# lucidrains/transfusion-pytorch

Measured on NVIDIA H100. Metric: train tokens/sec (text+latent) at d=512 L=8 seq=1024, higher is better.
Workload: dtype bf16

## Files before the change

transfusion_pytorch_b200/csrc/gemm_sm90.cuh:

```cuda
#pragma once
#include "sm90_ptx.cuh"
#include "dropout.cuh"

namespace tfx {

constexpr int GEMM_BM = 128;
constexpr int GEMM_BN = 128;
constexpr int GEMM_BK = 64;
constexpr int GEMM_UK = 16;

enum : int { EPI_STORE = 0, EPI_QKVG = 1, EPI_RESID = 2, EPI_GEGLU = 3, EPI_GEGLU_DROP = 4, EPI_QKVG_ROPE = 5 };

struct GemmParams {
  int M, N, K;
  int k_splits;
  float* out_f32; long long ld_f32;
  __nv_bfloat16* out_bf16; long long ld_bf16;
  const float* bias;
  const long long* row_off;
  float alpha;
  int accumulate_f32;
  int K1;
  int H;
  __nv_bfloat16 *q, *k, *v;
  float* gates;
  float* mix_pre;
  float* qk_inv;
  const float *q_gamma, *k_gamma;
  const int* rope_pos;
  const float2* rope_cs;
  int rope_len;
  const int* kv_rows;
  const float* x_res; float* x_out; __nv_bfloat16* x_out_bf16;
  __nv_bfloat16* y_bf16;
  const int* cond_row;
  const float* zgate;
  long long zgate_ld;
  const float* ls;
  __nv_bfloat16* vg;
  __nv_bfloat16* h;
  DropParams drop;
};

template <int EPI> struct GemmCfg {
  static constexpr int BM = GEMM_BM;
  static constexpr int THREADS = 384;
  static constexpr int STAGES = 4;
  static constexpr int A_BYTES = GEMM_BM * GEMM_BK * 2;
  static constexpr int B_BYTES = GEMM_BN * GEMM_BK * 2;
  static constexpr int STAGE_BYTES = A_BYTES + B_BYTES;
  static constexpr int ACC_BYTES = GEMM_BM * GEMM_BN * 4;
  static constexpr int STG_WARP = EPI == 2 ? 4096 + 2048 : 4096;
  static constexpr int STAGING = (EPI == EPI_GEGLU || EPI == EPI_GEGLU_DROP ? 8 : 4) * STG_WARP;
  static constexpr int SMEM_BYTES = STAGES * STAGE_BYTES + ACC_BYTES + STAGING + 1024  + 256 ;
  static_assert(SMEM_BYTES <= 227 * 1024, "shared memory of one block");
};

__device__ __forceinline__ uint32_t acc_off(int r, int col) { return r * 512 + ((((col >> 2) ^ (r & 7))) << 4) + (col & 3) * 4; }
__device__ __forceinline__ void acc_ld32(const uint8_t* acc, int r, int col, uint32_t (&v)[32]) {
#pragma unroll
  for (int q = 0; q < 8; ++q) {
    const uint4 t = *reinterpret_cast<const uint4*>(acc + r * 512 + ((((col >> 2) + q) ^ (r & 7)) << 4));
    v[4 * q] = t.x; v[4 * q + 1] = t.y; v[4 * q + 2] = t.z; v[4 * q + 3] = t.w;
  }
}

__device__ __forceinline__ void gelu_parts(float g, float& cdf, float& pdf) {
  const float ax = fabsf(g) * 0.70710678118654752f;
  const float t = __fdividef(1.f, fmaf(0.3275911f, ax, 1.f));
  const float E = __expf(-ax * ax);
  float poly = fmaf(1.061405429f, t, -1.453152027f);
  poly = fmaf(poly, t, 1.421413741f);
  poly = fmaf(poly, t, -0.284496736f);
  poly = fmaf(poly, t, 0.254829592f);
  const float h = 0.5f * poly * t * E;
  cdf = g >= 0.f ? 1.f - h : h;
  pdf = 0.3989422804014327f * E;
}
__device__ __forceinline__ float gelu_erf(float x) { float c, d; gelu_parts(x, c, d); return x * c; }
__device__ __forceinline__ float2 geglu_pair(float2 g, float2 v) {
  return make_float2(gelu_erf(g.x) * v.x, gelu_erf(g.y) * v.y);
}

__device__ __forceinline__ void cp_async16_zfill(void* smem, const void* gmem, bool valid) {
  const int sz = valid ? 16 : 0;
  asm volatile("cp.async.cg.shared.global [%0], [%1], 16, %2;" ::"r"(smem_u32(smem)), "l"(gmem), "r"(sz) : "memory");
}

__device__ __forceinline__ uint32_t pack_bf16(float a, float b) {
  __nv_bfloat162 t = __floats2bfloat162_rn(a, b);
  return *reinterpret_cast<uint32_t*>(&t);
}
__device__ __forceinline__ float2 unpack2_bf16_(uint32_t w) {
  __nv_bfloat162 t = *reinterpret_cast<__nv_bfloat162*>(&w);
  return __bfloat1622float2(t);
}

template <int CH>
__device__ __forceinline__ void stg_put(uint8_t* sw, int lane, const uint32_t* w) {
#pragma unroll
  for (int c = 0; c < CH; ++c)
    *reinterpret_cast<uint4*>(sw + lane * 128 + ((c ^ (lane & 7)) << 4)) = make_uint4(w[4 * c], w[4 * c + 1], w[4 * c + 2], w[4 * c + 3]);
}
template <int CH>
__device__ __forceinline__ void stg_get(const uint8_t* sw, int lane, uint32_t* w) {
#pragma unroll
  for (int c = 0; c < CH; ++c) {
    const uint4 t = *reinterpret_cast<const uint4*>(sw + lane * 128 + ((c ^ (lane & 7)) << 4));
    w[4 * c] = t.x; w[4 * c + 1] = t.y; w[4 * c + 2] = t.z; w[4 * c + 3] = t.w;
  }
}
template <int CH>
__device__ __forceinline__ void stg_store(const uint8_t* sw, int lane, uint8_t* g, long long pitch, int rows_valid) {
  constexpr int RPI = 32 / CH;
#pragma unroll
  for (int it = 0; it < 32 / RPI; ++it) {
    const int row = it * RPI + lane / CH, ch = lane % CH;
    if (row < rows_valid)
      *reinterpret_cast<uint4*>(g + row * pitch + ch * 16) = *reinterpret_cast<const uint4*>(sw + row * 128 + ((ch ^ (row & 7)) << 4));
  }
}
__device__ __forceinline__ void stg_fetch(int lane, const uint8_t* g, long long pitch, int rows_valid, uint4 (&t)[8]) {
#pragma unroll
  for (int it = 0; it < 8; ++it) {
    const int row = it * 4 + lane / 8, ch = lane % 8;
    t[it] = row < rows_valid ? *reinterpret_cast<const uint4*>(g + row * pitch + ch * 16) : make_uint4(0, 0, 0, 0);
  }
}
__device__ __forceinline__ void stg_fill(uint8_t* sw, int lane, const uint4 (&t)[8]) {
#pragma unroll
  for (int it = 0; it < 8; ++it) {
    const int row = it * 4 + lane / 8, ch = lane % 8;
    *reinterpret_cast<uint4*>(sw + row * 128 + ((ch ^ (row & 7)) << 4)) = t[it];
  }
}

__device__ __forceinline__ void stg_put_pack(uint8_t* sw, int lane, const float* y) {
#pragma unroll
  for (int c = 0; c < 4; ++c)
    *reinterpret_cast<uint4*>(sw + lane * 128 + ((c ^ (lane & 7)) << 4)) =
        make_uint4(pack_bf16(y[8 * c], y[8 * c + 1]), pack_bf16(y[8 * c + 2], y[8 * c + 3]), pack_bf16(y[8 * c + 4], y[8 * c + 5]), pack_bf16(y[8 * c + 6], y[8 * c + 7]));
}
__device__ __forceinline__ void stg64_put(uint8_t* sw, int lane, const uint32_t* w) {
#pragma unroll
  for (int c = 0; c < 4; ++c)
    *reinterpret_cast<uint4*>(sw + lane * 64 + ((c ^ ((lane >> 1) & 3)) << 4)) = make_uint4(w[4 * c], w[4 * c + 1], w[4 * c + 2], w[4 * c + 3]);
}
__device__ __forceinline__ void stg64_put_pack(uint8_t* sw, int lane, const float* y) {
#pragma unroll
  for (int c = 0; c < 4; ++c)
    *reinterpret_cast<uint4*>(sw + lane * 64 + ((c ^ ((lane >> 1) & 3)) << 4)) =
        make_uint4(pack_bf16(y[8 * c], y[8 * c + 1]), pack_bf16(y[8 * c + 2], y[8 * c + 3]), pack_bf16(y[8 * c + 4], y[8 * c + 5]), pack_bf16(y[8 * c + 6], y[8 * c + 7]));
}
__device__ __forceinline__ void stg64_store(const uint8_t* sw, int lane, uint8_t* g, long long pitch, int rows_valid) {
#pragma unroll
  for (int it = 0; it < 4; ++it) {
    const int row = it * 8 + (lane >> 2), ch = lane & 3;
    if (row < rows_valid)
      *reinterpret_cast<uint4*>(g + row * pitch + ch * 16) = *reinterpret_cast<const uint4*>(sw + row * 64 + ((ch ^ ((row >> 1) & 3)) << 4));
  }
}

__device__ __forceinline__ void stg64_store_rows(const uint8_t* sw, int lane, uint8_t* g, long long pitch, int rows_valid, const int* __restrict__ rows) {
#pragma unroll
  for (int it = 0; it < 4; ++it) {
    const int row = it * 8 + (lane >> 2), ch = lane & 3;
    if (row < rows_valid)
      *reinterpret_cast<uint4*>(g + (long long)rows[row] * pitch + ch * 16) = *reinterpret_cast<const uint4*>(sw + row * 64 + ((ch ^ ((row >> 1) & 3)) << 4));
  }
}
template <int CH>
__device__ __forceinline__ void stg_store_rows(const uint8_t* sw, int lane, uint8_t* g, long long pitch, int rows_valid, const int* __restrict__ rows) {
  constexpr int RPI = 32 / CH;
#pragma unroll
  for (int it = 0; it < 32 / RPI; ++it) {
    const int row = it * RPI + lane / CH, ch = lane % CH;
    if (row < rows_valid)
      *reinterpret_cast<uint4*>(g + (long long)rows[row] * pitch + ch * 16) = *reinterpret_cast<const uint4*>(sw + row * 128 + ((ch ^ (row & 7)) << 4));
  }
}

template <class RowOf>
__device__ __forceinline__ void store_slice(const GemmParams& p, uint8_t* sw, int lane, uint32_t (&r)[32], int cbase, RowOf row_of) {
  const bool f32_staged = p.out_f32 && (p.row_off || (p.ld_f32 & 3) == 0) && ((reinterpret_cast<uintptr_t>(p.out_f32) & 15) == 0);
  const bool bf16_staged = p.out_bf16 && (p.ld_bf16 & 7) == 0 && ((reinterpret_cast<uintptr_t>(p.out_bf16) & 15) == 0);
  const int row = row_of(lane);
  const bool row_ok = row < p.M;
  const bool full = cbase + 32 <= p.N;
  float v[32];
#pragma unroll
  for (int j = 0; j < 32; ++j) v[j] = __uint_as_float(r[j]);
  if (p.alpha != 1.f) {
#pragma unroll
    for (int j = 0; j < 32; ++j) v[j] *= p.alpha;
  }
  if (p.bias) {
    if (full) {
#pragma unroll
      for (int j = 0; j < 32; j += 4) { const float4 b = *reinterpret_cast<const float4*>(p.bias + cbase + j); v[j] += b.x; v[j + 1] += b.y; v[j + 2] += b.z; v[j + 3] += b.w; }
    } else {
      for (int j = 0; j < 32; ++j) if (cbase + j < p.N) v[j] += p.bias[cbase + j];
    }
  }
  if (p.out_f32) {
    if (full && f32_staged) {
#pragma unroll
      for (int j = 0; j < 32; ++j) r[j] = __float_as_uint(v[j]);
      stg_put<8>(sw, lane, r);
      __syncwarp();
      auto put = [&](float* dst, float x) { if (p.accumulate_f32) atomicAdd(dst, x); else *dst = x; };
#pragma unroll
      for (int it = 0; it < 8; ++it) {
        const int rr = it * 4 + (lane >> 3), ch = lane & 7;
        const int grow = row_of(rr);
        if (grow < p.M) {
          const long long off = p.row_off ? p.row_off[grow] : (long long)grow * p.ld_f32;
          if (off >= 0) {
            float* drow = p.out_f32 + off + cbase;
            const uint8_t* srow = sw + rr * 128;
            const int a = (int)(reinterpret_cast<uintptr_t>(drow) >> 2) & 3;
            if (a == 0) {
              float* dst = drow + ch * 4;
              const float4 t = *reinterpret_cast<const float4*>(srow + ((ch ^ (rr & 7)) << 4));
              if (p.accumulate_f32) asm volatile("red.global.add.v4.f32 [%0], {%1, %2, %3, %4};" ::"l"(dst), "f"(t.x), "f"(t.y), "f"(t.z), "f"(t.w) : "memory");
              else *reinterpret_cast<float4*>(dst) = t;
            } else {
              const int pe = 4 - a;
              auto col = [&](int j) { return *reinterpret_cast<const float*>(srow + (((j >> 2) ^ (rr & 7)) << 4) + (j & 3) * 4); };
              if (ch < 7) {
                const int j = pe + 4 * ch;
                float* dst = drow + j;
                const float4 t = make_float4(col(j), col(j + 1), col(j + 2), col(j + 3));
                if (p.accumulate_f32) asm volatile("red.global.add.v4.f32 [%0], {%1, %2, %3, %4};" ::"l"(dst), "f"(t.x), "f"(t.y), "f"(t.z), "f"(t.w) : "memory");
                else *reinterpret_cast<float4*>(dst) = t;
              } else {
#pragma unroll
                for (int i = 0; i < 4; ++i) { const int j = i < pe ? i : 28 + i; put(drow + j, col(j)); }
              }
            }
          }
        }
      }
      __syncwarp();
    } else if (row_ok) {
      const long long off = p.row_off ? p.row_off[row] : (long long)row * p.ld_f32;
      if (off >= 0) {
        float* dst = p.out_f32 + off + cbase;
        for (int j = 0; j < 32; ++j)
          if (cbase + j < p.N) { if (p.accumulate_f32) atomicAdd(dst + j, v[j]); else dst[j] = v[j]; }
      }
    }
  }
  if (p.out_bf16) {
    if (full && bf16_staged) {
      uint32_t w[16];
#pragma unroll
      for (int j = 0; j < 16; ++j) w[j] = pack_bf16(v[2 * j], v[2 * j + 1]);
      stg_put<4>(sw, lane, w);
      __syncwarp();
#pragma unroll
      for (int it = 0; it < 4; ++it) {
        const int rr = it * 8 + (lane >> 2), ch = lane & 3;
        const int grow = row_of(rr);
        if (grow < p.M)
          *reinterpret_cast<uint4*>(p.out_bf16 + (long long)grow * p.ld_bf16 + cbase + ch * 8) = *reinterpret_cast<const uint4*>(sw + rr * 128 + ((ch ^ (rr & 7)) << 4));
      }
      __syncwarp();
    } else if (row_ok) {
      __nv_bfloat16* dst = p.out_bf16 + (long long)row * p.ld_bf16 + cbase;
      for (int j = 0; j < 32; ++j) if (cbase + j < p.N) dst[j] = __float2bfloat16(v[j]);
    }
  }
}

template <int BM, int CL>
struct GemmSched {
  struct Work { int m_blk, n_blk, kb0, kb1; };
  int n_tiles, unit_items, kb_total, kb_per_split, num_items;
  __device__ __forceinline__ explicit GemmSched(const GemmParams& p) {
    const int m_tiles = (p.M + BM - 1) / BM;
    n_tiles = (p.N + GEMM_BN - 1) / GEMM_BN;
    kb_total = (p.K + GEMM_BK - 1) / GEMM_BK;
    kb_per_split = (kb_total + p.k_splits - 1) / p.k_splits;
    unit_items = (m_tiles + CL - 1) / CL * n_tiles;
    num_items = unit_items * p.k_splits;
  }
  __device__ __forceinline__ Work work(int item, int cta_rank) const {
    const int split = item / unit_items;
    const int rem = item - split * unit_items;
    const int m_unit = rem / n_tiles;
    const int kb0 = split * kb_per_split;
    return {m_unit * CL + cta_rank, rem - m_unit * n_tiles, kb0, min(kb0 + kb_per_split, kb_total)};
  }
};

template <int STAGES>
struct GemmRing {
  int stage = 0; uint32_t phase = 0;
  __device__ __forceinline__ void step() { if (++stage == STAGES) { stage = 0; phase ^= 1; } }
};

template <class Cfg, bool A_MN, bool B_MN, int CL, bool TWO_A>
__device__ __forceinline__ void gemm_fill(uint8_t* smem, uint64_t* full_bar, uint64_t* empty_bar, GemmRing<Cfg::STAGES>& ring,
                                          const CUtensorMap* tmA, const CUtensorMap* tmA2, const CUtensorMap* tmB, const GemmParams& p,
                                          int kb, int m_blk, int n_blk, int cta_rank) {
  constexpr int BM = Cfg::BM, BN = GEMM_BN;
  mbar_wait(&empty_bar[ring.stage], ring.phase ^ 1);
  uint8_t* sA = smem + ring.stage * Cfg::STAGE_BYTES;
  uint8_t* sB = sA + Cfg::A_BYTES;
  uint64_t* bar = &full_bar[ring.stage];
  mbar_expect_tx(bar, Cfg::STAGE_BYTES);
  if (!A_MN) {
    if (!TWO_A || kb * GEMM_BK < p.K1) tma_load_2d(tmA, bar, sA, kb * GEMM_BK, m_blk * BM);
    else tma_load_2d(tmA2, bar, sA, kb * GEMM_BK - p.K1, m_blk * BM);
  } else {
#pragma unroll
    for (int a = 0; a < BM / 64; ++a)
      tma_load_2d(tmA, bar, sA + a * (GEMM_BK * 128), m_blk * BM + a * 64, kb * GEMM_BK);
  }
  if constexpr (CL > 1) {
    if (!B_MN) tma_load_2d_multicast(tmB, bar, sB + cta_rank * (64 * 128), kb * GEMM_BK, n_blk * BN + cta_rank * 64, (uint16_t)3);
    else tma_load_2d_multicast(tmB, bar, sB + cta_rank * (GEMM_BK * 128), n_blk * BN + cta_rank * 64, kb * GEMM_BK, (uint16_t)3);
  } else if (!B_MN) {
    tma_load_2d(tmB, bar, sB, kb * GEMM_BK, n_blk * BN);
  } else {
#pragma unroll
    for (int a = 0; a < BN / 64; ++a)
      tma_load_2d(tmB, bar, sB + a * (GEMM_BK * 128), n_blk * BN + a * 64, kb * GEMM_BK);
  }
  ring.step();
}

template <class Cfg, bool A_MN, bool B_MN, class Release>
__device__ __forceinline__ int gemm_mainloop(uint8_t* smem, uint64_t* full_bar, GemmRing<Cfg::STAGES>& ring, uint32_t a_off, int kb0, int kb1,
                                             float (&d0)[64], float (&d1)[64], Release& release) {
#pragma unroll
  for (int i = 0; i < 64; ++i) { d0[i] = 0.f; d1[i] = 0.f; }
  int prev_stage = -1;
  for (int kb = kb0; kb < kb1; ++kb) {
    mbar_wait(&full_bar[ring.stage], ring.phase);
    const uint32_t sA = smem_u32(smem + ring.stage * Cfg::STAGE_BYTES) + a_off;
    const uint32_t sB = smem_u32(smem + ring.stage * Cfg::STAGE_BYTES) + Cfg::A_BYTES;
    wgmma_reg_fence(d0);
    wgmma_reg_fence(d1);
    wgmma_fence();
#pragma unroll
    for (int k = 0; k < GEMM_BK / GEMM_UK; ++k) {
      const uint64_t db = B_MN ? wgmma_desc_sw128(sB + k * (GEMM_UK * 128), GEMM_BK * 128, 1024)
                               : wgmma_desc_sw128(sB + k * (GEMM_UK * 2), 16, 1024);
      const uint64_t da0 = A_MN ? wgmma_desc_sw128(sA + k * (GEMM_UK * 128), GEMM_BK * 128, 1024)
                                : wgmma_desc_sw128(sA + k * (GEMM_UK * 2), 16, 1024);
      const uint64_t da1 = A_MN ? wgmma_desc_sw128(sA + GEMM_BK * 128 + k * (GEMM_UK * 128), GEMM_BK * 128, 1024)
                                : wgmma_desc_sw128(sA + 64 * 128 + k * (GEMM_UK * 2), 16, 1024);
      const uint32_t acc_flag = (kb > kb0 || k > 0) ? 1u : 0u;
      wgmma_m64n128_ss<A_MN ? 1 : 0, B_MN ? 1 : 0>(d0, da0, db, acc_flag);
      wgmma_m64n128_ss<A_MN ? 1 : 0, B_MN ? 1 : 0>(d1, da1, db, acc_flag);
    }
    wgmma_commit();
    wgmma_wait<1>();
    if (prev_stage >= 0) release(prev_stage);
    prev_stage = ring.stage;
    ring.step();
  }
  return prev_stage;
}

template <class Release>
__device__ __forceinline__ void gemm_drain(float (&d0)[64], float (&d1)[64], int last_stage, Release& release) {
  wgmma_wait<0>();
  wgmma_reg_fence(d0);
  wgmma_reg_fence(d1);
  if (last_stage >= 0) release(last_stage);
}

template <bool A_MN, bool B_MN, int EPI, int CL>
__global__ void __launch_bounds__(384, 1)
gemm_sm90_kernel(const __grid_constant__ CUtensorMap tmA, const __grid_constant__ CUtensorMap tmA2, const __grid_constant__ CUtensorMap tmB, const GemmParams p) {
  using Cfg = GemmCfg<EPI>;
  constexpr bool GEGLU = EPI == EPI_GEGLU || EPI == EPI_GEGLU_DROP;
  constexpr int BN = GEMM_BN;
  constexpr int STAGES = Cfg::STAGES;
  static_assert(Cfg::STAGE_BYTES % 1024 == 0 && 2 * STAGES <= 32, "stage alignment / barrier area");
  extern __shared__ __align__(1024) uint8_t smem_raw[];
  uint8_t* smem = smem_raw;
  if (threadIdx.x == 0 && (smem_u32(smem) & 1023u) != 0) __trap();
  uint8_t* acc = smem + STAGES * Cfg::STAGE_BYTES;
  uint8_t* staging = acc + Cfg::ACC_BYTES;
  uint64_t* bars = reinterpret_cast<uint64_t*>(staging + Cfg::STAGING);
  uint64_t* full_bar = bars;
  uint64_t* empty_bar = bars + STAGES;

  const int warp = threadIdx.x >> 5, lane = threadIdx.x & 31;
  const GemmSched<GEMM_BM, CL> sched(p);
  const int num_items = sched.num_items;
  const int cta_rank = CL > 1 ? (int)cluster_ctarank() : 0;
  const int first_item = blockIdx.x / CL, item_stride = gridDim.x / CL;

  if (threadIdx.x == 0) {
    tma_prefetch_desc(&tmA);
    tma_prefetch_desc(&tmB);
    for (int s = 0; s < STAGES; ++s) { mbar_init(&full_bar[s], 1); mbar_init(&empty_bar[s], 4 * CL); }
    mbar_fence_init();
  }
  __syncthreads();
  if constexpr (CL > 1) cluster_sync_all();

  if (warp < 4) {
    setmaxnreg_dec<40>();
    if (threadIdx.x == 0) {
      GemmRing<STAGES> ring;
      for (int item = first_item; item < num_items; item += item_stride) {
        const auto w = sched.work(item, cta_rank);
        for (int kb = w.kb0; kb < w.kb1; ++kb)
          gemm_fill<Cfg, A_MN, B_MN, CL, true>(smem, full_bar, empty_bar, ring, &tmA, &tmA2, &tmB, p, kb, w.m_blk, w.n_blk, cta_rank);
      }
    }
  } else {
    setmaxnreg_inc<232>();
    constexpr int BAR_TILE = 1, BAR_MMA = 3, BAR_ACC = 5;
    const int cw = (warp >> 2) - 1;
    const int quad = warp & 3;
    uint8_t* sw = staging + ((GEGLU ? 4 * cw : 0) + quad) * Cfg::STG_WARP;
    const int erow = quad * 32 + lane;
    GemmRing<STAGES> ring;
    auto release = [&](int s) {
      __syncwarp();
      if (lane == 0) {
        if constexpr (CL > 1) { mbar_arrive_cluster(&empty_bar[s], 0); mbar_arrive_cluster(&empty_bar[s], 1); }
        else mbar_arrive(&empty_bar[s]);
      }
    };
    int nth = 0;
    for (int item = first_item; item < num_items; item += item_stride, ++nth) {
      const auto [m_blk, n_blk, kb0, kb1] = sched.work(item, cta_rank);
      if ((nth & 1) != cw) {
        const int s = ring.stage + (kb1 - kb0);
        ring.stage = s % STAGES;
        ring.phase ^= (uint32_t)(s / STAGES) & 1u;
        continue;
      }
      const bool has_next = item + item_stride < num_items;
      if (nth > 0) named_bar_sync(BAR_MMA + cw, 256);
      float d0[64], d1[64];
      const int last_stage = gemm_mainloop<Cfg, A_MN, B_MN>(smem, full_bar, ring, 0, kb0, kb1, d0, d1, release);
      if (has_next) named_bar_arrive(BAR_MMA + (cw ^ 1), 256);
      gemm_drain(d0, d1, last_stage, release);

      if (nth > 0) named_bar_sync(BAR_ACC + cw, 256);
      {
        const int r0 = quad * 16 + (lane >> 2);
#pragma unroll
        for (int q = 0; q < 16; ++q) {
          const int c = 8 * q + 2 * (lane & 3);
          *reinterpret_cast<float2*>(acc + acc_off(r0, c)) = make_float2(d0[4 * q], d0[4 * q + 1]);
          *reinterpret_cast<float2*>(acc + acc_off(r0 + 8, c)) = make_float2(d0[4 * q + 2], d0[4 * q + 3]);
          *reinterpret_cast<float2*>(acc + acc_off(r0 + 64, c)) = make_float2(d1[4 * q], d1[4 * q + 1]);
          *reinterpret_cast<float2*>(acc + acc_off(r0 + 72, c)) = make_float2(d1[4 * q + 2], d1[4 * q + 3]);
        }
      }
      named_bar_sync(BAR_TILE + cw, 128);

      const int wrow0 = m_blk * GEMM_BM + quad * 32;
      const int row = wrow0 + lane;
      const bool row_ok = row < p.M;
      const int rows_valid = min(32, p.M - wrow0);
      const int col0 = n_blk * BN;
      int qk_pos = 0;
      if constexpr (EPI == EPI_QKVG || EPI == EPI_QKVG_ROPE) { qk_pos = row_ok ? p.rope_pos[row] : 0; }
      if constexpr (EPI == EPI_RESID) { qk_pos = (row_ok && p.cond_row) ? p.cond_row[row] : -1; }

      if constexpr (EPI == EPI_STORE) {
#pragma unroll 1
        for (int c = 0; c < BN / 32; ++c) {
          const int cbase = col0 + c * 32;
          if (cbase >= p.N) break;
          uint32_t r[32];
          acc_ld32(acc, erow, c * 32, r);
          store_slice(p, sw, lane, r, cbase, [&](int i) { return wrow0 + i; });
        }
      } else if constexpr (EPI == EPI_QKVG || EPI == EPI_QKVG_ROPE) {
        const int tps = p.H >> 1;
        const int kind = n_blk / tps;
        const int tis = n_blk - kind * tps;
        const long long HI = (long long)p.H * 64;
        if (kind <= 1) {
          const float* gamma = kind == 0 ? p.q_gamma : p.k_gamma;
          __nv_bfloat16* dstm = kind == 0 ? p.q : p.k;
          const float2* cs = p.rope_cs + qk_pos;
#pragma unroll
          for (int hh = 0; hh < 2; ++hh) {
            uint32_t r0[32], r1[32];
            acc_ld32(acc, erow, hh * 64, r0);
            acc_ld32(acc, erow, hh * 64 + 32, r1);
            float sc = 1.f;
            if constexpr (EPI == EPI_QKVG) {
              float ss = 0.f;
#pragma unroll
              for (int j = 0; j < 32; ++j) { float a = __uint_as_float(r0[j]), b = __uint_as_float(r1[j]); ss += a * a + b * b; }
              const float inv = 1.f / fmaxf(sqrtf(ss), 1e-12f);
              if (row_ok) p.qk_inv[(long long)row * 2 * p.H + kind * p.H + tis * 2 + hh] = inv;
              sc = inv * 8.f;
            }
            const int head = tis * 2 + hh;
            uint32_t outw[32];
#pragma unroll
            for (int dh = 0; dh < 2; ++dh) {
              uint32_t* rr = dh == 0 ? r0 : r1;
#pragma unroll
              for (int i = 0; i < 16; ++i) {
                const int d0 = dh * 32 + 2 * i;
                float y0 = __uint_as_float(rr[2 * i]), y1 = __uint_as_float(rr[2 * i + 1]);
                if constexpr (EPI == EPI_QKVG) {
                  const float2 gm = *reinterpret_cast<const float2*>(gamma + d0);
                  y0 = y0 * sc * (gm.x + 1.f);
                  y1 = y1 * sc * (gm.y + 1.f);
                }
                const float2 cc = cs[(long long)(dh * 16 + i) * p.rope_len];
                outw[dh * 16 + i] = pack_bf16(y0 * cc.x - y1 * cc.y, y1 * cc.x + y0 * cc.y);
              }
            }
            stg_put<8>(sw, lane, outw);
            __syncwarp();
            if (kind == 1 && p.kv_rows) stg_store_rows<8>(sw, lane, reinterpret_cast<uint8_t*>(dstm + head * 64), HI * 2, rows_valid, p.kv_rows + wrow0);
            else stg_store<8>(sw, lane, reinterpret_cast<uint8_t*>(dstm + (long long)wrow0 * HI + head * 64), HI * 2, rows_valid);
            __syncwarp();
          }
        } else if (kind == 2) {
#pragma unroll
          for (int c = 0; c < 2; ++c) {
            uint32_t r0[32], r1[32], w[32];
            acc_ld32(acc, erow, c * 64, r0);
            acc_ld32(acc, erow, c * 64 + 32, r1);
#pragma unroll
            for (int j = 0; j < 16; ++j) {
              w[j] = pack_bf16(__uint_as_float(r0[2 * j]), __uint_as_float(r0[2 * j + 1]));
              w[16 + j] = pack_bf16(__uint_as_float(r1[2 * j]), __uint_as_float(r1[2 * j + 1]));
            }
            stg_put<8>(sw, lane, w);
            __syncwarp();
            if (p.kv_rows) stg_store_rows<8>(sw, lane, reinterpret_cast<uint8_t*>(p.v + tis * 128 + c * 64), HI * 2, rows_valid, p.kv_rows + wrow0);
            else stg_store<8>(sw, lane, reinterpret_cast<uint8_t*>(p.v + (long long)wrow0 * HI + tis * 128 + c * 64), HI * 2, rows_valid);
            __syncwarp();
          }
        } else {
          uint32_t r[32];
          acc_ld32(acc, erow, 0, r);
          if (row_ok) {
            float* dst = p.gates + (long long)row * p.H;
#pragma unroll
            for (int j = 0; j < 32; ++j) if (j < p.H) dst[j] = __uint_as_float(r[j]);
            if (p.mix_pre) {
              float* dm = p.mix_pre + (long long)row * p.H;
#pragma unroll
              for (int j = 0; j < 32; ++j) if (j >= p.H && j < 2 * p.H) dm[j - p.H] = __uint_as_float(r[j]);
            }
          }
        }
      } else if constexpr (EPI == EPI_RESID) {
        const int crow = qk_pos;
        const float* zrow = (p.zgate && crow >= 0) ? p.zgate + (long long)crow * p.zgate_ld : nullptr;
        uint8_t* swb = sw + 4096;
        uint4 xres[8];
        auto fetch = [&](int sl) {
          stg_fetch(lane, reinterpret_cast<const uint8_t*>(p.x_res + (long long)wrow0 * p.N + col0 + sl * 32), (long long)p.N * 4,
                    col0 + sl * 32 < p.N ? rows_valid : 0, xres);
        };
        fetch(0);
#pragma unroll 1
        for (int sl = 0; sl < BN / 32; ++sl) {
          const int cbase = col0 + sl * 32;
          if (cbase >= p.N) break;
          __syncwarp();
          stg_fill(sw, lane, xres);
          if (sl + 1 < BN / 32) fetch(sl + 1);
          uint32_t r[32];
          acc_ld32(acc, erow, sl * 32, r);
          float y[32];
#pragma unroll
          for (int j = 0; j < 32; ++j) y[j] = __uint_as_float(r[j]);
          if (p.bias) {
#pragma unroll
            for (int j = 0; j < 32; j += 4) { const float4 b = *reinterpret_cast<const float4*>(p.bias + cbase + j); y[j] += b.x; y[j + 1] += b.y; y[j + 2] += b.z; y[j + 3] += b.w; }
          }
          if (p.y_bf16) {
            stg64_put_pack(swb, lane, y);
            __syncwarp();
            stg64_store(swb, lane, reinterpret_cast<uint8_t*>(p.y_bf16 + (long long)wrow0 * p.N + cbase), (long long)p.N * 2, rows_valid);
            __syncwarp();
          }
          {
            uint32_t xrv[32];
            __syncwarp();
            stg_get<8>(sw, lane, xrv);
            if (zrow) {
#pragma unroll
              for (int j = 0; j < 32; j += 4) {
                const float4 s4 = *reinterpret_cast<const float4*>(zrow + cbase + j);
                y[j] = __uint_as_float(xrv[j]) + y[j] * s4.x; y[j + 1] = __uint_as_float(xrv[j + 1]) + y[j + 1] * s4.y;
                y[j + 2] = __uint_as_float(xrv[j + 2]) + y[j + 2] * s4.z; y[j + 3] = __uint_as_float(xrv[j + 3]) + y[j + 3] * s4.w;
              }
            } else if (p.ls) {
#pragma unroll
              for (int j = 0; j < 32; j += 4) {
                const float4 s4 = *reinterpret_cast<const float4*>(p.ls + cbase + j);
                y[j] = __uint_as_float(xrv[j]) + y[j] * (s4.x + 1.f); y[j + 1] = __uint_as_float(xrv[j + 1]) + y[j + 1] * (s4.y + 1.f);
                y[j + 2] = __uint_as_float(xrv[j + 2]) + y[j + 2] * (s4.z + 1.f); y[j + 3] = __uint_as_float(xrv[j + 3]) + y[j + 3] * (s4.w + 1.f);
              }
            } else {
#pragma unroll
              for (int j = 0; j < 32; ++j) y[j] += __uint_as_float(xrv[j]);
            }
          }
          if (p.x_out)
#pragma unroll
          for (int hfc = 0; hfc < 2; ++hfc) {
            uint32_t w16[16];
#pragma unroll
            for (int j = 0; j < 16; ++j) w16[j] = __float_as_uint(y[hfc * 16 + j]);
            __syncwarp();
            stg64_put(swb, lane, w16);
            __syncwarp();
            stg64_store(swb, lane, reinterpret_cast<uint8_t*>(p.x_out + (long long)wrow0 * p.N + cbase + hfc * 16), (long long)p.N * 4, rows_valid);
          }
          if (p.x_out_bf16) {
            __syncwarp();
            stg64_put_pack(swb, lane, y);
            __syncwarp();
            stg64_store(swb, lane, reinterpret_cast<uint8_t*>(p.x_out_bf16 + (long long)wrow0 * p.N + cbase), (long long)p.N * 2, rows_valid);
          }
          __syncwarp();
        }
      } else if constexpr (GEGLU) {
        uint32_t keep[2] = {0u, 0u};
        if constexpr (EPI == EPI_GEGLU_DROP) {
          const uint32_t k0 = __ldg(p.drop.key), k1 = __ldg(p.drop.key + 1);
#pragma unroll
          for (int q = 0; q < 8; ++q) keep[q >> 2] |= drop_keep8(p.drop, k0, k1, DROP_SITE_FFN, 0, (uint32_t)row, (uint32_t)(n_blk * 8 + q)) << (8 * (q & 3));
        }
        uint32_t ra[4][32];
#pragma unroll
        for (int q = 0; q < 4; ++q) acc_ld32(acc, erow, q * 32, ra[q]);
        if (has_next) named_bar_arrive(BAR_ACC + (cw ^ 1), 256);
#pragma unroll
        for (int c = 0; c < 2; ++c) {
          const int cv = col0 + c * 32, cg = cv + 64;
          if (cv >= p.N) break;
          float v[32], g[32];
#pragma unroll
          for (int j = 0; j < 32; ++j) { v[j] = __uint_as_float(ra[c][j]) + p.bias[cv + j]; g[j] = __uint_as_float(ra[2 + c][j]) + p.bias[cg + j]; }
          __syncwarp();
          stg64_put_pack(sw, lane, v);
          __syncwarp();
          stg64_store(sw, lane, reinterpret_cast<uint8_t*>(p.vg + (long long)wrow0 * p.N + cv), (long long)p.N * 2, rows_valid);
          __syncwarp();
          stg64_put_pack(sw, lane, g);
          __syncwarp();
          stg64_store(sw, lane, reinterpret_cast<uint8_t*>(p.vg + (long long)wrow0 * p.N + cg), (long long)p.N * 2, rows_valid);
#pragma unroll
          for (int j = 0; j < 32; j += 2) {
            const float2 o = geglu_pair(make_float2(g[j], g[j + 1]), make_float2(v[j], v[j + 1]));
            g[j] = o.x; g[j + 1] = o.y;
          }
          if constexpr (EPI == EPI_GEGLU_DROP) {
#pragma unroll
            for (int j = 0; j < 32; ++j) g[j] = (keep[c] >> j) & 1u ? g[j] * p.drop.scale : 0.f;
          }
          __syncwarp();
          stg64_put_pack(sw, lane, g);
          __syncwarp();
          stg64_store(sw, lane, reinterpret_cast<uint8_t*>(p.h + (long long)wrow0 * (p.N / 2) + n_blk * 64 + c * 32), (long long)p.N, rows_valid);
          __syncwarp();
        }
      }
      if (!GEGLU && has_next) named_bar_arrive(BAR_ACC + (cw ^ 1), 256);
    }
  }
  if constexpr (CL > 1) {
    __syncthreads();
    cluster_sync_all();
  }
}

struct GemmWideCfg {
  static constexpr int BM = 256;
  static constexpr int THREADS = 384;
  static constexpr int STAGES = 4;
  static constexpr int A_BYTES = BM * GEMM_BK * 2;
  static constexpr int B_BYTES = GEMM_BN * GEMM_BK * 2;
  static constexpr int STAGE_BYTES = A_BYTES + B_BYTES;
  static constexpr int STAGING = 8 * 4096;
  static constexpr int SMEM_BYTES = STAGES * STAGE_BYTES + STAGING + 1024  + 256 ;
  static_assert(SMEM_BYTES <= 227 * 1024, "shared memory of one block");
};

template <bool A_MN, bool B_MN>
__global__ void __launch_bounds__(384, 1)
gemm_sm90_wide_kernel(const __grid_constant__ CUtensorMap tmA, const __grid_constant__ CUtensorMap tmB, const GemmParams p) {
  using Cfg = GemmWideCfg;
  constexpr int BM = Cfg::BM, BN = GEMM_BN, STAGES = Cfg::STAGES;
  static_assert(Cfg::STAGE_BYTES % 1024 == 0, "stage alignment");
  extern __shared__ __align__(1024) uint8_t smem_raw[];
  uint8_t* smem = smem_raw;
  if (threadIdx.x == 0 && (smem_u32(smem) & 1023u) != 0) __trap();
  uint8_t* staging = smem + STAGES * Cfg::STAGE_BYTES;
  uint64_t* full_bar = reinterpret_cast<uint64_t*>(staging + Cfg::STAGING);
  uint64_t* empty_bar = full_bar + STAGES;

  const int warp = threadIdx.x >> 5, lane = threadIdx.x & 31;
  const GemmSched<BM, 1> sched(p);
  const int num_items = sched.num_items;

  if (threadIdx.x == 0) {
    tma_prefetch_desc(&tmA);
    tma_prefetch_desc(&tmB);
    for (int s = 0; s < STAGES; ++s) { mbar_init(&full_bar[s], 1); mbar_init(&empty_bar[s], 8); }
    mbar_fence_init();
  }
  __syncthreads();

  if (warp < 4) {
    setmaxnreg_dec<40>();
    if (threadIdx.x == 0) {
      GemmRing<STAGES> ring;
      for (int item = blockIdx.x; item < num_items; item += gridDim.x) {
        const auto w = sched.work(item, 0);
        for (int kb = w.kb0; kb < w.kb1; ++kb)
          gemm_fill<Cfg, A_MN, B_MN, 1, false>(smem, full_bar, empty_bar, ring, &tmA, nullptr, &tmB, p, kb, w.m_blk, w.n_blk, 0);
      }
    }
  } else {
    setmaxnreg_inc<232>();
    const int cw = (warp >> 2) - 1;
    const int quad = warp & 3;
    uint8_t* sw = staging + (4 * cw + quad) * 4096;
    const uint32_t a_half = (uint32_t)cw * (A_MN ? 2 * GEMM_BK * 128 : 128 * 128);
    GemmRing<STAGES> ring;
    auto release = [&](int s) { __syncwarp(); if (lane == 0) mbar_arrive(&empty_bar[s]); };
    for (int item = blockIdx.x; item < num_items; item += gridDim.x) {
      const auto [m_blk, n_blk, kb0, kb1] = sched.work(item, 0);
      float d0[64], d1[64];
      const int last_stage = gemm_mainloop<Cfg, A_MN, B_MN>(smem, full_bar, ring, a_half, kb0, kb1, d0, d1, release);
      gemm_drain(d0, d1, last_stage, release);

      const int wrow0 = m_blk * BM + 128 * cw + 16 * quad;
      const int r0 = lane >> 2;
#pragma unroll
      for (int c = 0; c < BN / 32; ++c) {
        const int cbase = n_blk * BN + c * 32;
        if (cbase >= p.N) break;
#pragma unroll
        for (int q4 = 0; q4 < 4; ++q4) {
          const int q = 4 * c + q4, col = 8 * q4 + 2 * (lane & 3);
          auto put2 = [&](int rr, float x, float y) {
            *reinterpret_cast<float2*>(sw + rr * 128 + ((((col >> 2) ^ (rr & 7))) << 4) + (col & 3) * 4) = make_float2(x, y);
          };
          put2(r0, d0[4 * q], d0[4 * q + 1]);
          put2(r0 + 8, d0[4 * q + 2], d0[4 * q + 3]);
          put2(r0 + 16, d1[4 * q], d1[4 * q + 1]);
          put2(r0 + 24, d1[4 * q + 2], d1[4 * q + 3]);
        }
        __syncwarp();
        uint32_t r[32];
        stg_get<8>(sw, lane, r);
        __syncwarp();
        store_slice(p, sw, lane, r, cbase, [&](int i) { return wrow0 + (i & 15) + ((i >> 4) << 6); });
      }
    }
  }
}

typedef CUresult (*PFN_encodeTiled)(CUtensorMap*, CUtensorMapDataType, cuuint32_t, void*, const cuuint64_t*, const cuuint64_t*,
                                    const cuuint32_t*, const cuuint32_t*, CUtensorMapInterleave, CUtensorMapSwizzle,
                                    CUtensorMapL2promotion, CUtensorMapFloatOOBfill);

inline PFN_encodeTiled get_encode_fn() {
  static PFN_encodeTiled fn = nullptr;
  if (!fn) {
    void* f = nullptr;
    cudaDriverEntryPointQueryResult qres;
    if (cudaGetDriverEntryPoint("cuTensorMapEncodeTiled", &f, cudaEnableDefault, &qres) != cudaSuccess || !f) return nullptr;
    fn = reinterpret_cast<PFN_encodeTiled>(f);
  }
  return fn;
}

inline int make_tmap_bf16(CUtensorMap* tm, const void* ptr, long long inner, long long outer, long long ld, int box_rows) {
  PFN_encodeTiled enc = get_encode_fn();
  if (!enc) return -1;
  cuuint64_t dims[2] = {(cuuint64_t)inner, (cuuint64_t)outer};
  cuuint64_t strides[1] = {(cuuint64_t)ld * 2};
  cuuint32_t box[2] = {64, (cuuint32_t)box_rows};
  cuuint32_t estr[2] = {1, 1};
  CUresult r = enc(tm, CU_TENSOR_MAP_DATA_TYPE_BFLOAT16, 2, const_cast<void*>(ptr), dims, strides, box, estr,
                   CU_TENSOR_MAP_INTERLEAVE_NONE, CU_TENSOR_MAP_SWIZZLE_128B, CU_TENSOR_MAP_L2_PROMOTION_L2_256B,
                   CU_TENSOR_MAP_FLOAT_OOB_FILL_NONE);
  return r == CUDA_SUCCESS ? 0 : -(int)r - 1000;
}

struct GemmOperand {
  const void* ptr;
  long long ld;
  bool mn_major;
  const void* ptr2 = nullptr;
  long long ld2 = 0;
};

inline int make_operand_tmap(CUtensorMap* tm, const GemmOperand& X, long long mn, long long k, int box_rows) {
  return X.mn_major ? make_tmap_bf16(tm, X.ptr, mn, k, X.ld, GEMM_BK) : make_tmap_bf16(tm, X.ptr, k, mn, X.ld, box_rows);
}

template <class Cfg, auto kern, class... Args>
int launch_persistent(int items, int num_sms, cudaStream_t stream, const Args&... args) {
  static bool attr_set = false;
  if (!attr_set) {
    if (cudaFuncSetAttribute(kern, cudaFuncAttributeMaxDynamicSharedMemorySize, Cfg::SMEM_BYTES) != cudaSuccess) return -2;
    attr_set = true;
  }
  const int grid = items < num_sms ? items : num_sms;
  kern<<<grid, Cfg::THREADS, Cfg::SMEM_BYTES, stream>>>(args...);
  return cudaGetLastError() == cudaSuccess ? 0 : -3;
}

inline int& gemm_cluster_mode_ref() {
  static int mode = -1;
  if (mode < 0) { const char* e = getenv("TFX_GEMM_CLUSTER"); mode = e ? atoi(e) : 1; }
  return mode;
}

inline int gemm_effective_splits(int K, int k_splits) {
  const int kbt = (K + GEMM_BK - 1) / GEMM_BK;
  int s = k_splits < 1 ? 1 : k_splits > kbt ? kbt : k_splits;
  const int per = (kbt + s - 1) / s;
  return (kbt + per - 1) / per;
}
inline int gemm_kb_per_item(int K, int k_splits) { return ((K + GEMM_BK - 1) / GEMM_BK + k_splits - 1) / k_splits; }

constexpr int GEMM_WIDE_MIN_KB = 16;
inline int& gemm_wide_mode_ref() { static int mode = 1; return mode; }
inline bool gemm_store_wide(int K, int k_splits) {
  const int mode = gemm_wide_mode_ref();
  if (mode != 1) return mode == 2;
  return gemm_cluster_mode_ref() == 1 && gemm_kb_per_item(K, gemm_effective_splits(K, k_splits)) >= GEMM_WIDE_MIN_KB;
}

template <bool A_MN, bool B_MN>
int launch_gemm_wide_t(const GemmOperand& A, const GemmOperand& B, const GemmParams& p_in, int num_sms, cudaStream_t stream) {
  using Cfg = GemmWideCfg;
  GemmParams p = p_in;
  p.K1 = p.K;
  p.k_splits = gemm_effective_splits(p.K, p.k_splits);
  const int items = ((p.M + Cfg::BM - 1) / Cfg::BM) * ((p.N + GEMM_BN - 1) / GEMM_BN) * p.k_splits;
  if (items <= 0) return 0;
  CUtensorMap tmA, tmB;
  int rc = make_operand_tmap(&tmA, A, p.M, p.K, Cfg::BM);
  if (rc) return rc;
  rc = make_operand_tmap(&tmB, B, p.N, p.K, GEMM_BN);
  if (rc) return rc;
  return launch_persistent<Cfg, gemm_sm90_wide_kernel<A_MN, B_MN>>(items, num_sms, stream, tmA, tmB, p);
}

template <bool A_MN, bool B_MN, int EPI>
int launch_gemm_t(const GemmOperand& A, const GemmOperand& B, const GemmParams& p_in, int num_sms, cudaStream_t stream) {
  using Cfg = GemmCfg<EPI>;
  GemmParams p = p_in;
  CUtensorMap tmA, tmA2, tmB;
  const bool two = (!A_MN) && A.ptr2 != nullptr;
  if (!two) p.K1 = p.K;
  int rc = make_operand_tmap(&tmA, A, p.M, p.K1, GEMM_BM);
  if (rc) return rc;
  if (two) { rc = make_tmap_bf16(&tmA2, A.ptr2, p.K - p.K1, p.M, A.ld2, GEMM_BM); if (rc) return rc; } else tmA2 = tmA;
  p.k_splits = gemm_effective_splits(p.K, p.k_splits);
  const int m_tiles = (p.M + GEMM_BM - 1) / GEMM_BM, n_tiles = (p.N + GEMM_BN - 1) / GEMM_BN;
  const int items = m_tiles * n_tiles * p.k_splits;
  if (items <= 0) return 0;
  const int mode = gemm_cluster_mode_ref();
  const int kb_item = gemm_kb_per_item(p.K, p.k_splits);
  const bool paired = mode == 2 || (mode == 3 && m_tiles >= 2 && kb_item >= 16 && items >= 2 * num_sms);
  rc = make_operand_tmap(&tmB, B, p.N, p.K, paired ? GEMM_BN / 2 : GEMM_BN);
  if (rc) return rc;
  if (paired) {
    auto kern = gemm_sm90_kernel<A_MN, B_MN, EPI, 2>;
    static int max_clusters = 0;
    cudaLaunchConfig_t cfg;
    memset(&cfg, 0, sizeof(cfg));
    cudaLaunchAttribute at[1];
    at[0].id = cudaLaunchAttributeClusterDimension;
    at[0].val.clusterDim.x = 2; at[0].val.clusterDim.y = 1; at[0].val.clusterDim.z = 1;
    cfg.blockDim = dim3(Cfg::THREADS); cfg.dynamicSmemBytes = Cfg::SMEM_BYTES; cfg.stream = stream; cfg.attrs = at; cfg.numAttrs = 1;
    if (!max_clusters) {
      if (cudaFuncSetAttribute(kern, cudaFuncAttributeMaxDynamicSharedMemorySize, Cfg::SMEM_BYTES) != cudaSuccess) return -2;
      cfg.gridDim = dim3(2 * (num_sms / 2));
      int nc = 0;
      if (cudaOccupancyMaxActiveClusters(&nc, kern, &cfg) != cudaSuccess || nc < 1) { cudaGetLastError(); nc = num_sms / 2; }
      max_clusters = nc < num_sms / 2 ? nc : num_sms / 2;
    }
    const int pair_items = ((m_tiles + 1) / 2) * n_tiles * p.k_splits;
    const int clusters = pair_items < max_clusters ? pair_items : max_clusters;
    cfg.gridDim = dim3(2 * clusters);
    return cudaLaunchKernelEx(&cfg, kern, tmA, tmA2, tmB, p) == cudaSuccess ? 0 : -3;
  }
  return launch_persistent<Cfg, gemm_sm90_kernel<A_MN, B_MN, EPI, 1>>(items, num_sms, stream, tmA, tmA2, tmB, p);
}

}
```

transfusion_pytorch_b200/csrc/sm90_ptx.cuh:

```cuda
#pragma once
#include <cuda.h>
#include <cuda_runtime.h>
#include <cuda_bf16.h>
#include <stdint.h>
#include <stdio.h>

namespace tfx {

#ifndef TFX_SPIN_LIMIT
#define TFX_SPIN_LIMIT (1u << 24)
#endif

__device__ __forceinline__ uint32_t smem_u32(const void* p) {
  return static_cast<uint32_t>(__cvta_generic_to_shared(p));
}

__device__ __forceinline__ void mbar_init(uint64_t* bar, uint32_t count) {
  asm volatile("mbarrier.init.shared::cta.b64 [%0], %1;" ::"r"(smem_u32(bar)), "r"(count));
}
__device__ __forceinline__ void mbar_fence_init() {
  asm volatile("fence.mbarrier_init.release.cluster;" ::: "memory");
}
__device__ __forceinline__ void mbar_expect_tx(uint64_t* bar, uint32_t bytes) {
  asm volatile("mbarrier.arrive.expect_tx.shared::cta.b64 _, [%0], %1;" ::"r"(smem_u32(bar)), "r"(bytes) : "memory");
}
__device__ __forceinline__ void mbar_arrive(uint64_t* bar) {
  asm volatile("mbarrier.arrive.shared::cta.b64 _, [%0];" ::"r"(smem_u32(bar)) : "memory");
}
__device__ __forceinline__ bool mbar_try_wait(uint64_t* bar, uint32_t parity) {
  uint32_t ok;
  asm volatile(
      "{\n\t.reg .pred p;\n\t"
      "mbarrier.try_wait.parity.shared::cta.b64 p, [%1], %2;\n\t"
      "selp.u32 %0, 1, 0, p;\n\t}"
      : "=r"(ok) : "r"(smem_u32(bar)), "r"(parity) : "memory");
  return ok != 0;
}
__device__ __forceinline__ void mbar_wait(uint64_t* bar, uint32_t parity) {
  uint32_t spins = 0;
  while (!mbar_try_wait(bar, parity)) {
    if (++spins > TFX_SPIN_LIMIT) {
#if defined(TFX_DEBUG_SPIN) && TFX_DEBUG_SPIN
      printf("tfx: mbarrier timeout block %d thread %d bar %u parity %u\n", blockIdx.x, threadIdx.x, smem_u32(bar), parity);
#endif
      __trap();
    }
  }
}

__device__ __forceinline__ void tma_prefetch_desc(const CUtensorMap* m) {
  asm volatile("prefetch.tensormap [%0];" ::"l"(reinterpret_cast<uint64_t>(m)) : "memory");
}
__device__ __forceinline__ void tma_load_2d(const CUtensorMap* m, uint64_t* bar, void* smem, int c0, int c1) {
  asm volatile(
      "cp.async.bulk.tensor.2d.shared::cluster.global.mbarrier::complete_tx::bytes [%0], [%1, {%3, %4}], [%2];"
      ::"r"(smem_u32(smem)), "l"(reinterpret_cast<uint64_t>(m)), "r"(smem_u32(bar)), "r"(c0), "r"(c1)
      : "memory");
}
__device__ __forceinline__ void tma_load_1d(const CUtensorMap* m, uint64_t* bar, void* smem, int c0) {
  asm volatile(
      "cp.async.bulk.tensor.1d.shared::cluster.global.mbarrier::complete_tx::bytes [%0], [%1, {%3}], [%2];"
      ::"r"(smem_u32(smem)), "l"(reinterpret_cast<uint64_t>(m)), "r"(smem_u32(bar)), "r"(c0)
      : "memory");
}
__device__ __forceinline__ void tma_reduce_add_2d(const CUtensorMap* m, const void* smem, int c0, int c1) {
  asm volatile("cp.reduce.async.bulk.tensor.2d.global.shared::cta.add.tile.bulk_group [%0, {%2, %3}], [%1];"
               ::"l"(reinterpret_cast<uint64_t>(m)), "r"(smem_u32(smem)), "r"(c0), "r"(c1) : "memory");
}
__device__ __forceinline__ void bulk_commit() { asm volatile("cp.async.bulk.commit_group;" ::: "memory"); }
__device__ __forceinline__ void bulk_wait_read_all() { asm volatile("cp.async.bulk.wait_group.read 0;" ::: "memory"); }
__device__ __forceinline__ void bulk_wait_all() { asm volatile("cp.async.bulk.wait_group 0;" ::: "memory"); }
__device__ __forceinline__ void tma_load_2d_multicast(const CUtensorMap* m, uint64_t* bar, void* smem, int c0, int c1, uint16_t mask) {
  asm volatile(
      "cp.async.bulk.tensor.2d.shared::cluster.global.mbarrier::complete_tx::bytes.multicast::cluster [%0], [%1, {%3, %4}], [%2], %5;"
      ::"r"(smem_u32(smem)), "l"(reinterpret_cast<uint64_t>(m)), "r"(smem_u32(bar)), "r"(c0), "r"(c1), "h"(mask)
      : "memory");
}
__device__ __forceinline__ uint32_t cluster_ctarank() { uint32_t r; asm volatile("mov.u32 %0, %%cluster_ctarank;" : "=r"(r)); return r; }
__device__ __forceinline__ void cluster_sync_all() {
  asm volatile("barrier.cluster.arrive.release.aligned;\n\tbarrier.cluster.wait.acquire.aligned;" ::: "memory");
}
__device__ __forceinline__ void mbar_arrive_cluster(uint64_t* bar, uint32_t rank) {
  uint32_t remote;
  asm volatile("mapa.shared::cluster.u32 %0, %1, %2;" : "=r"(remote) : "r"(smem_u32(bar)), "r"(rank));
  asm volatile("mbarrier.arrive.release.cluster.shared::cluster.b64 _, [%0];" ::"r"(remote) : "memory");
}
__device__ __forceinline__ void fence_proxy_async_smem() {
  asm volatile("fence.proxy.async.shared::cta;" ::: "memory");
}
__device__ __forceinline__ void named_bar_sync(int id, int count) {
  asm volatile("bar.sync %0, %1;" ::"r"(id), "r"(count) : "memory");
}
__device__ __forceinline__ void named_bar_arrive(int id, int count) {
  asm volatile("bar.arrive %0, %1;" ::"r"(id), "r"(count) : "memory");
}

template <int N> __device__ __forceinline__ void setmaxnreg_dec() { asm volatile("setmaxnreg.dec.sync.aligned.u32 %0;" ::"n"(N)); }
template <int N> __device__ __forceinline__ void setmaxnreg_inc() { asm volatile("setmaxnreg.inc.sync.aligned.u32 %0;" ::"n"(N)); }

__device__ __forceinline__ void wgmma_fence() { asm volatile("wgmma.fence.sync.aligned;" ::: "memory"); }
__device__ __forceinline__ void wgmma_commit() { asm volatile("wgmma.commit_group.sync.aligned;" ::: "memory"); }
template <int N> __device__ __forceinline__ void wgmma_wait() { asm volatile("wgmma.wait_group.sync.aligned %0;" ::"n"(N) : "memory"); }
template <int N> __device__ __forceinline__ void wgmma_reg_fence(float (&d)[N]) {
#pragma unroll
  for (int i = 0; i < N; ++i) asm volatile("" : "+f"(d[i])::"memory");
}

template <int TA, int TB>
__device__ __forceinline__ void wgmma_m64n128_ss(float (&d)[64], uint64_t da, uint64_t db, uint32_t accumulate) {
  asm volatile(
      "{\n\t.reg .pred p;\n\t"
      "setp.ne.b32 p, %66, 0;\n\t"
      "wgmma.mma_async.sync.aligned.m64n128k16.f32.bf16.bf16 "
      "{%0, %1, %2, %3, %4, %5, %6, %7, %8, %9, %10, %11, %12, %13, %14, %15, %16, %17, %18, %19, %20, %21, %22, %23, %24, %25, %26, %27, %28, %29, %30, %31, %32, %33, %34, %35, %36, %37, %38, %39, %40, %41, %42, %43, %44, %45, %46, %47, %48, %49, %50, %51, %52, %53, %54, %55, %56, %57, %58, %59, %60, %61, %62, %63}, "
      "%64, %65, p, 1, 1, %67, %68;\n\t}"
      : "+f"(d[0]), "+f"(d[1]), "+f"(d[2]), "+f"(d[3]), "+f"(d[4]), "+f"(d[5]), "+f"(d[6]), "+f"(d[7]), "+f"(d[8]), "+f"(d[9]), "+f"(d[10]), "+f"(d[11]), "+f"(d[12]), "+f"(d[13]), "+f"(d[14]), "+f"(d[15]), "+f"(d[16]), "+f"(d[17]), "+f"(d[18]), "+f"(d[19]), "+f"(d[20]), "+f"(d[21]), "+f"(d[22]), "+f"(d[23]), "+f"(d[24]), "+f"(d[25]), "+f"(d[26]), "+f"(d[27]), "+f"(d[28]), "+f"(d[29]), "+f"(d[30]), "+f"(d[31]), "+f"(d[32]), "+f"(d[33]), "+f"(d[34]), "+f"(d[35]), "+f"(d[36]), "+f"(d[37]), "+f"(d[38]), "+f"(d[39]), "+f"(d[40]), "+f"(d[41]), "+f"(d[42]), "+f"(d[43]), "+f"(d[44]), "+f"(d[45]), "+f"(d[46]), "+f"(d[47]), "+f"(d[48]), "+f"(d[49]), "+f"(d[50]), "+f"(d[51]), "+f"(d[52]), "+f"(d[53]), "+f"(d[54]), "+f"(d[55]), "+f"(d[56]), "+f"(d[57]), "+f"(d[58]), "+f"(d[59]), "+f"(d[60]), "+f"(d[61]), "+f"(d[62]), "+f"(d[63])
      : "l"(da), "l"(db), "r"(accumulate), "n"(TA), "n"(TB));
}
template <int TA, int TB>
__device__ __forceinline__ void wgmma_m64n64_ss(float (&d)[32], uint64_t da, uint64_t db, uint32_t accumulate) {
  asm volatile(
      "{\n\t.reg .pred p;\n\t"
      "setp.ne.b32 p, %34, 0;\n\t"
      "wgmma.mma_async.sync.aligned.m64n64k16.f32.bf16.bf16 "
      "{%0, %1, %2, %3, %4, %5, %6, %7, %8, %9, %10, %11, %12, %13, %14, %15, %16, %17, %18, %19, %20, %21, %22, %23, %24, %25, %26, %27, %28, %29, %30, %31}, "
      "%32, %33, p, 1, 1, %35, %36;\n\t}"
      : "+f"(d[0]), "+f"(d[1]), "+f"(d[2]), "+f"(d[3]), "+f"(d[4]), "+f"(d[5]), "+f"(d[6]), "+f"(d[7]), "+f"(d[8]), "+f"(d[9]), "+f"(d[10]), "+f"(d[11]), "+f"(d[12]), "+f"(d[13]), "+f"(d[14]), "+f"(d[15]), "+f"(d[16]), "+f"(d[17]), "+f"(d[18]), "+f"(d[19]), "+f"(d[20]), "+f"(d[21]), "+f"(d[22]), "+f"(d[23]), "+f"(d[24]), "+f"(d[25]), "+f"(d[26]), "+f"(d[27]), "+f"(d[28]), "+f"(d[29]), "+f"(d[30]), "+f"(d[31])
      : "l"(da), "l"(db), "r"(accumulate), "n"(TA), "n"(TB));
}
template <int TB>
__device__ __forceinline__ void wgmma_m64n64_rs(float (&d)[32], const uint32_t (&a)[4], uint64_t db, uint32_t accumulate) {
  asm volatile(
      "{\n\t.reg .pred p;\n\t"
      "setp.ne.b32 p, %37, 0;\n\t"
      "wgmma.mma_async.sync.aligned.m64n64k16.f32.bf16.bf16 "
      "{%0, %1, %2, %3, %4, %5, %6, %7, %8, %9, %10, %11, %12, %13, %14, %15, %16, %17, %18, %19, %20, %21, %22, %23, %24, %25, %26, %27, %28, %29, %30, %31}, "
      "{%32, %33, %34, %35}, %36, p, 1, 1, %38;\n\t}"
      : "+f"(d[0]), "+f"(d[1]), "+f"(d[2]), "+f"(d[3]), "+f"(d[4]), "+f"(d[5]), "+f"(d[6]), "+f"(d[7]), "+f"(d[8]), "+f"(d[9]), "+f"(d[10]), "+f"(d[11]), "+f"(d[12]), "+f"(d[13]), "+f"(d[14]), "+f"(d[15]), "+f"(d[16]), "+f"(d[17]), "+f"(d[18]), "+f"(d[19]), "+f"(d[20]), "+f"(d[21]), "+f"(d[22]), "+f"(d[23]), "+f"(d[24]), "+f"(d[25]), "+f"(d[26]), "+f"(d[27]), "+f"(d[28]), "+f"(d[29]), "+f"(d[30]), "+f"(d[31])
      : "r"(a[0]), "r"(a[1]), "r"(a[2]), "r"(a[3]), "l"(db), "r"(accumulate), "n"(TB));
}

__device__ __forceinline__ uint64_t wgmma_desc_sw128(uint32_t smem_addr, uint32_t lbo_bytes, uint32_t sbo_bytes) {
  uint64_t d = 0;
  d |= (uint64_t)((smem_addr >> 4) & 0x3FFF);
  d |= (uint64_t)((lbo_bytes >> 4) & 0x3FFF) << 16;
  d |= (uint64_t)((sbo_bytes >> 4) & 0x3FFF) << 32;
  d |= (uint64_t)1 << 62;
  return d;
}

}
```

Measured before the change: 1.235 million.

## Compute GEGLU epilogue from wgmma fragments and store tiles via TMA

```diff
diff --git a/transfusion_pytorch_b200/csrc/gemm_sm90.cuh b/transfusion_pytorch_b200/csrc/gemm_sm90.cuh
--- a/transfusion_pytorch_b200/csrc/gemm_sm90.cuh
+++ b/transfusion_pytorch_b200/csrc/gemm_sm90.cuh
@@ -43,16 +43,19 @@
 };
 
 template <int EPI> struct GemmCfg {
+  static constexpr bool FRAG = EPI == EPI_GEGLU;
   static constexpr int BM = GEMM_BM;
   static constexpr int THREADS = 384;
   static constexpr int STAGES = 4;
   static constexpr int A_BYTES = GEMM_BM * GEMM_BK * 2;
   static constexpr int B_BYTES = GEMM_BN * GEMM_BK * 2;
   static constexpr int STAGE_BYTES = A_BYTES + B_BYTES;
-  static constexpr int ACC_BYTES = GEMM_BM * GEMM_BN * 4;
+  static constexpr int ACC_BYTES = FRAG ? 0 : GEMM_BM * GEMM_BN * 4;
   static constexpr int STG_WARP = EPI == 2 ? 4096 + 2048 : 4096;
-  static constexpr int STAGING = (EPI == EPI_GEGLU || EPI == EPI_GEGLU_DROP ? 8 : 4) * STG_WARP;
-  static constexpr int SMEM_BYTES = STAGES * STAGE_BYTES + ACC_BYTES + STAGING + 1024  + 256 ;
+  static constexpr int STAGING = FRAG ? 0 : (EPI == EPI_GEGLU_DROP ? 8 : 4) * STG_WARP;
+  static constexpr int OUT_BOX = GEMM_BM * 128;
+  static constexpr int OUT_BYTES = FRAG ? 2 * 3 * OUT_BOX : 0;
+  static constexpr int SMEM_BYTES = STAGES * STAGE_BYTES + ACC_BYTES + STAGING + OUT_BYTES + 1024  + 256 ;
   static_assert(SMEM_BYTES <= 227 * 1024, "shared memory of one block");
 };
 
@@ -373,11 +376,16 @@
   if (last_stage >= 0) release(last_stage);
 }
 
+template <bool ON> struct FragOutMaps { CUtensorMap vg, h; };
+template <> struct FragOutMaps<false> {};
+
 template <bool A_MN, bool B_MN, int EPI, int CL>
 __global__ void __launch_bounds__(384, 1)
-gemm_sm90_kernel(const __grid_constant__ CUtensorMap tmA, const __grid_constant__ CUtensorMap tmA2, const __grid_constant__ CUtensorMap tmB, const GemmParams p) {
+gemm_sm90_kernel(const __grid_constant__ CUtensorMap tmA, const __grid_constant__ CUtensorMap tmA2, const __grid_constant__ CUtensorMap tmB,
+                 const __grid_constant__ FragOutMaps<GemmCfg<EPI>::FRAG> tmO, const GemmParams p) {
   using Cfg = GemmCfg<EPI>;
   constexpr bool GEGLU = EPI == EPI_GEGLU || EPI == EPI_GEGLU_DROP;
+  constexpr bool FRAG = Cfg::FRAG;
   constexpr int BN = GEMM_BN;
   constexpr int STAGES = Cfg::STAGES;
   static_assert(Cfg::STAGE_BYTES % 1024 == 0 && 2 * STAGES <= 32, "stage alignment / barrier area");
@@ -386,7 +394,8 @@
   if (threadIdx.x == 0 && (smem_u32(smem) & 1023u) != 0) __trap();
   uint8_t* acc = smem + STAGES * Cfg::STAGE_BYTES;
   uint8_t* staging = acc + Cfg::ACC_BYTES;
-  uint64_t* bars = reinterpret_cast<uint64_t*>(staging + Cfg::STAGING);
+  uint8_t* out_tiles = staging + Cfg::STAGING;
+  uint64_t* bars = reinterpret_cast<uint64_t*>(out_tiles + Cfg::OUT_BYTES);
   uint64_t* full_bar = bars;
   uint64_t* empty_bar = bars + STAGES;
 
@@ -399,6 +408,7 @@
   if (threadIdx.x == 0) {
     tma_prefetch_desc(&tmA);
     tma_prefetch_desc(&tmB);
+    if constexpr (FRAG) { tma_prefetch_desc(&tmO.vg); tma_prefetch_desc(&tmO.h); }
     for (int s = 0; s < STAGES; ++s) { mbar_init(&full_bar[s], 1); mbar_init(&empty_bar[s], 4 * CL); }
     mbar_fence_init();
   }
@@ -421,6 +431,8 @@
     const int cw = (warp >> 2) - 1;
     const int quad = warp & 3;
     uint8_t* sw = staging + ((GEGLU ? 4 * cw : 0) + quad) * Cfg::STG_WARP;
+    uint8_t* ot = out_tiles + cw * 3 * Cfg::OUT_BOX;
+    const bool out_leader = quad == 0 && lane == 0;
     const int erow = quad * 32 + lane;
     GemmRing<STAGES> ring;
     auto release = [&](int s) {
@@ -445,6 +457,41 @@
       const int last_stage = gemm_mainloop<Cfg, A_MN, B_MN>(smem, full_bar, ring, 0, kb0, kb1, d0, d1, release);
       if (has_next) named_bar_arrive(BAR_MMA + (cw ^ 1), 256);
       gemm_drain(d0, d1, last_stage, release);
+
+      if constexpr (FRAG) {
+        if (out_leader) bulk_wait_read_all();
+        named_bar_sync(BAR_TILE + cw, 128);
+        const int col0 = n_blk * BN;
+#pragma unroll
+        for (int q = 0; q < 8; ++q) {
+          const int c = 8 * q + 2 * (lane & 3);
+          const float2 bv = make_float2(p.bias[col0 + c], p.bias[col0 + c + 1]);
+          const float2 bg = make_float2(p.bias[col0 + 64 + c], p.bias[col0 + 64 + c + 1]);
+#pragma unroll
+          for (int e = 0; e < 4; ++e) {
+            const int rr = 16 * quad + (lane >> 2) + 8 * (e & 1) + 64 * (e >> 1);
+            const float* d = e >> 1 ? d1 : d0;
+            const int i = 2 * (e & 1);
+            const float2 v = make_float2(d[4 * q + i] + bv.x, d[4 * q + i + 1] + bv.y);
+            const float2 g = make_float2(d[4 * (q + 8) + i] + bg.x, d[4 * (q + 8) + i + 1] + bg.y);
+            const float2 o = geglu_pair(g, v);
+            const uint32_t off = rr * 128 + ((((c >> 3) ^ (rr & 7))) << 4) + (c & 7) * 2;
+            *reinterpret_cast<uint32_t*>(ot + off) = pack_bf16(v.x, v.y);
+            *reinterpret_cast<uint32_t*>(ot + Cfg::OUT_BOX + off) = pack_bf16(g.x, g.y);
+            *reinterpret_cast<uint32_t*>(ot + 2 * Cfg::OUT_BOX + off) = pack_bf16(o.x, o.y);
+          }
+        }
+        fence_proxy_async_smem();
+        named_bar_sync(BAR_TILE + cw, 128);
+        if (out_leader) {
+          tma_store_2d(&tmO.vg, ot, col0, m_blk * GEMM_BM);
+          tma_store_2d(&tmO.vg, ot + Cfg::OUT_BOX, col0 + 64, m_blk * GEMM_BM);
+          tma_store_2d(&tmO.h, ot + 2 * Cfg::OUT_BOX, n_blk * 64, m_blk * GEMM_BM);
+          bulk_commit();
+        }
+        __syncwarp();
+        continue;
+      }
 
       if (nth > 0) named_bar_sync(BAR_ACC + cw, 256);
       {
@@ -674,6 +721,7 @@
       }
       if (!GEGLU && has_next) named_bar_arrive(BAR_ACC + (cw ^ 1), 256);
     }
+    if constexpr (FRAG) { if (out_leader) bulk_wait_read_all(); }
   }
   if constexpr (CL > 1) {
     __syncthreads();
@@ -878,6 +926,13 @@
   const bool paired = mode == 2 || (mode == 3 && m_tiles >= 2 && kb_item >= 16 && items >= 2 * num_sms);
   rc = make_operand_tmap(&tmB, B, p.N, p.K, paired ? GEMM_BN / 2 : GEMM_BN);
   if (rc) return rc;
+  FragOutMaps<Cfg::FRAG> tmO;
+  if constexpr (Cfg::FRAG) {
+    rc = make_tmap_bf16(&tmO.vg, p.vg, p.N, p.M, p.N, GEMM_BM);
+    if (rc) return rc;
+    rc = make_tmap_bf16(&tmO.h, p.h, p.N / 2, p.M, p.N / 2, GEMM_BM);
+    if (rc) return rc;
+  }
   if (paired) {
     auto kern = gemm_sm90_kernel<A_MN, B_MN, EPI, 2>;
     static int max_clusters = 0;
@@ -897,9 +952,9 @@
     const int pair_items = ((m_tiles + 1) / 2) * n_tiles * p.k_splits;
     const int clusters = pair_items < max_clusters ? pair_items : max_clusters;
     cfg.gridDim = dim3(2 * clusters);
-    return cudaLaunchKernelEx(&cfg, kern, tmA, tmA2, tmB, p) == cudaSuccess ? 0 : -3;
-  }
-  return launch_persistent<Cfg, gemm_sm90_kernel<A_MN, B_MN, EPI, 1>>(items, num_sms, stream, tmA, tmA2, tmB, p);
-}
-
-}
+    return cudaLaunchKernelEx(&cfg, kern, tmA, tmA2, tmB, tmO, p) == cudaSuccess ? 0 : -3;
+  }
+  return launch_persistent<Cfg, gemm_sm90_kernel<A_MN, B_MN, EPI, 1>>(items, num_sms, stream, tmA, tmA2, tmB, tmO, p);
+}
+
+}
diff --git a/transfusion_pytorch_b200/csrc/sm90_ptx.cuh b/transfusion_pytorch_b200/csrc/sm90_ptx.cuh
--- a/transfusion_pytorch_b200/csrc/sm90_ptx.cuh
+++ b/transfusion_pytorch_b200/csrc/sm90_ptx.cuh
@@ -65,6 +65,10 @@
 }
 __device__ __forceinline__ void tma_reduce_add_2d(const CUtensorMap* m, const void* smem, int c0, int c1) {
   asm volatile("cp.reduce.async.bulk.tensor.2d.global.shared::cta.add.tile.bulk_group [%0, {%2, %3}], [%1];"
+               ::"l"(reinterpret_cast<uint64_t>(m)), "r"(smem_u32(smem)), "r"(c0), "r"(c1) : "memory");
+}
+__device__ __forceinline__ void tma_store_2d(const CUtensorMap* m, const void* smem, int c0, int c1) {
+  asm volatile("cp.async.bulk.tensor.2d.global.shared::cta.bulk_group [%0, {%2, %3}], [%1];"
                ::"l"(reinterpret_cast<uint64_t>(m)), "r"(smem_u32(smem)), "r"(c0), "r"(c1) : "memory");
 }
 __device__ __forceinline__ void bulk_commit() { asm volatile("cp.async.bulk.commit_group;" ::: "memory"); }
```

Result: no change. 1.244 million, median of 6 (+0.8%).
